# GimpelZhang/GaussianRPG

Measured on AMD Instinct MI355X. Metric: frames/sec @1920x1280, ~2M Gaussians; achieved HBM GB/s vs peak, higher is better.
Workload: dtype f32; 1 GPU; configs[2]: scene-002-like synthetic street scene (seed 2), forward op + clamp + uint8 pack per frame, 200-pose drive, frames sharded round-robin over ranks; P=2000000, width=1920, height=1280, sh_degree=1, M=4, S=0, streams_per_gpu=3, binning_mode=speculative, binning_algorithm=hierarchical, entry_point=GaussianRasterizer.forward, deferred_count=False, frames_rendered_twice=0, parallelism=replicas x1, frame-sharded, final uint8 gather

## Files before the change

### gaussianrpg_amd/csrc/api.hip

```cpp
#include <hip/hip_runtime.h>

#include <atomic>
#include <cmath>
#include <sys/syscall.h>
#include <unistd.h>

#include <cstdio>
#include <cstdlib>
#include <cstring>
#include <mutex>
#include <string>
#include <functional>
#include <vector>

#include "../../include/grpg_rasterizer.h"
#include "abi_util.h"
#include "common.h"

using namespace grpg;

static thread_local std::string g_last_error;

namespace grpg {

// ... 206 lines not shown

int check_async_error(HostWord* hw) {
  if (hw && hw->host_ptr[3] != 0u) {
    hw->host_ptr[3] = 0u;
    return fail(GRPG_ERR_HIP, "render: a producer/consumer hand-over timed out in an earlier frame "
                              "of this thread (image blob header pc_timeout): that frame's image is invalid");
  }
  return GRPG_OK;
}

std::atomic<int> g_binning_alg{[] {
  const char* e = getenv("GRPG_BINNING");
  return (e && strcmp(e, "sort") == 0) ? GRPG_BINNING_ALG_SORT : GRPG_BINNING_ALG_HIER;
}()};
bool binning_is_hier() { return g_binning_alg.load() == GRPG_BINNING_ALG_HIER; }

int bits_for(uint32_t T) {
  int b = 0;
  while ((1ull << b) < (unsigned long long)T) b++;
  return b;
}

struct TimingRecord {
  hipEvent_t ev[GRPG_NUM_STAGES + 1];
  int stage_of[GRPG_NUM_STAGES + 1];
  int n = 0;
};
thread_local std::vector<TimingRecord*> g_pending;
thread_local std::vector<TimingRecord*> g_free;

// ... 413 lines not shown
  uint32_t* const tiles_sorted = (uint32_t*)(geom + GL.tiles_sorted);
  uint32_t* const emit_win = (uint32_t*)(geom + GL.emit_win);
  uint2* const rect_sorted = (uint2*)(geom + GL.rect_sorted);
  uint4* const pre_counts = (uint4*)(geom + GL.pre_counts);
  BlobHeader* const gh = (BlobHeader*)geom;
  uint2* const ranges = (uint2*)(img + IL.ranges);
  uint32_t* const n_contrib = (uint32_t*)(img + IL.n_contrib);
  uint32_t* const work = (uint32_t*)(img + IL.work);

  const bool spec_mode = g_binning_mode.load() == GRPG_BINNING_SPECULATIVE;
  const bool fat_sort = depth_sort_is_fat(GL.nchunks_ds);
  const uint32_t NS = super_tiles(cam.gx, cam.gy);
  const bool hier = fat_sort && binning_is_hier() && NS <= 65536u;
  const bool rect_sorted_by_sort = hier && cam.gx <= 255 && cam.gy <= 255;
  uint2* const rects = hier ? (uint2*)(geom + GL.rects) : nullptr;
  const bool with_ckpt = training && q.S == 0;
  const LayerArgs* const layers = q.layers;
  unsigned char* const tile_obj = layers ? (unsigned char*)(img + IL.ck_count) : nullptr;
  const uint32_t tile_obj_words = layers ? (T + 3u) / 4u : 0u;
  const TileClasses frame_classes = layers ? tile_classes_layers(tile_obj, cam.gx) : tile_classes(q.S);
  const LayerMarks marks = {layers ? layers->layer_class : nullptr, tile_obj, cam.gx};

  const FrameEpilogue* epi = q.epi;
  FrameEpilogue epi_drained;
  uint32_t drain_cnt_words = 0u;
  StageTimer tm{stream, g_timing_enabled};

  HostWord* hw = nullptr;
  uint32_t* pub_ptr = nullptr;
  const uint32_t* pub_host = nullptr;
  hipEvent_t pub_ev = nullptr;
  CapKey ck{-1, 0, 0, 0};
  bool speculative = false;
  bool with_pass3 = true;
  char* bin = nullptr;
// ... 83 lines not shown
    launch_compose_features(stream, q.P, seg_dev, fdev, q.nseg, q.feat_S, q.feat_normals, q.cam_pos,
                            (float*)(q.feat_blob + FL.features));
    return GRPG_OK;
  }

  int enqueue_head() {
    tm.mark(0);
    launch_frame_init(stream, geom, bin, img, (uint32_t)q.P, fat_sort ? 0u : (uint32_t)q.P, Rcap,
                      (uint32_t)q.width, (uint32_t)q.height, (uint32_t)q.S, ranges, T, work,
                      geom + GL.zero_begin, GL.zero_end - GL.zero_begin, training,
                      drain_cnt_words ? (uint32_t*)(img + IL.ck_count) : (uint32_t*)tile_obj,
                      drain_cnt_words ? T + drain_cnt_words : tile_obj_words);
    if (q.segs == nullptr) {
      launch_preprocess(stream, q.P, q.D, q.M, q.means3D, q.scales, q.scale_modifier, q.rotations, q.opacities,
                        q.shs, q.cov3D_precomp, q.colors_precomp, cam, radii_int, rec_w, key_a, tiles, rects,
                        fat_sort ? ds_table : nullptr, pre_counts, marks);
    } else {
      SegmentDev* seg_dev = (SegmentDev*)(geom + GL.seg_table);
      if (int rc = stage_segments(seg_dev)) return rc;
      launch_preprocess_composed(stream, q.P, q.D, q.M, seg_dev, q.nseg, q.scale_modifier, cam, radii_int, rec_w,
                                 key_a, tiles, rects, fat_sort ? ds_table : nullptr, pre_counts, marks);
      if (q.S > 0) {
        if (int rc = stage_features(seg_dev)) return rc;
      }
    }
    const bool fold_publish = fat_sort;
    if (!fold_publish) {
      launch_publish_counts(stream, pre_counts, (uint32_t)((q.P + 255) / 256), pub_ptr, &gh->R_pre);
      HIP_TRY(hipEventRecord(pub_ev, stream));
    }
    STAGE_CHECK("preprocess");
    tm.mark(1);
    if (fat_sort) {
      const uint32_t pnb = (uint32_t)((q.P + 255) / 256);
      uint32_t* key_c = (uint32_t*)(geom + GL.key_c);
      uint32_t* val_c = (uint32_t*)(geom + GL.val_c);
// ... 992 lines not shown
                      const char* binning_buffer, const char* image_buffer, uint64_t* keys_sorted,
                      uint32_t* point_list, uint32_t* ranges, uint32_t* n_contrib, float* means2D,
                      float* depths, float* conic_opacity, float* rgb, uint32_t* tiles_touched,
                      void* hip_stream) {
  if (int rc = begin_call()) return rc;
  if (P < 0 || R < 0 || !geom_buffer || !binning_buffer || !image_buffer)
    return fail(GRPG_ERR_INVALID_ARGUMENT, "bad argument");
  hipStream_t stream = (hipStream_t)hip_stream;
  const int gx = (width + TILE - 1) / TILE, gy = (height + TILE - 1) / TILE;
  const GeomLayout GL = geom_layout((size_t)P);
  BlobHeader bh;
  HIP_TRY(hipMemcpyAsync(&bh, binning_buffer, sizeof(BlobHeader), hipMemcpyDeviceToHost, stream));
  HIP_TRY(hipStreamSynchronize(stream));
  if (bh.magic != BIN_MAGIC || bh.Rcap < (uint32_t)R)
    return fail(GRPG_ERR_BAD_BUFFER, "binning buffer does not match this call");
  const BinLayout BL = bh.hier ? bin_layout((size_t)bh.Rcap, (size_t)gx * gy, super_tiles(gx, gy), (size_t)bh.Rc)
                               : bin_layout((size_t)bh.Rcap);
  const ImgLayout IL = img_layout((size_t)gx * gy, (size_t)width * height);
  launch_debug_export(stream, P, (uint32_t)R, width, height, gx, gy,
                      RecView{(const float4*)(geom_buffer + GL.rec)},
                      (const uint32_t*)(geom_buffer + GL.tiles),
                      (const uint32_t*)(binning_buffer + BL.key_a),
                      bh.hier ? (const uint32_t*)(binning_buffer + BL.tile_start) : nullptr,
                      (const uint32_t*)(binning_buffer + BL.val_a),
                      (const uint2*)(image_buffer + IL.ranges),
                      (const uint32_t*)(image_buffer + IL.n_contrib), keys_sorted, point_list,
                      ranges, n_contrib, means2D, depths, conic_opacity, rgb, tiles_touched);
  HIP_TRY(hipGetLastError());
  return GRPG_OK;
}

}
```

### gaussianrpg_amd/csrc/blend_math.h

```cpp
#pragma once
#include "common.h"

namespace grpg {

typedef float v2f __attribute__((ext_vector_type(2)));

constexpr float LOG2E = 1.4426950408889634f;
constexpr float ALPHA_MIN = 1.0f / 255.0f;
constexpr float ALPHA_MAX = 0.99f;

struct SplatQ {
  float A, B, C;
};

__device__ __forceinline__ SplatQ splat_q(const float cx, const float cy, const float cz) {
  SplatQ q;
  q.A = (-0.5f * LOG2E) * cx;
  q.B = (-LOG2E) * cy;
  q.C = (-0.5f * LOG2E) * cz;
  return q;
}

__device__ __forceinline__ bool splat_power_never_positive(const SplatQ q) {
  const float a = -q.A, c = -q.C;
// ... 55 lines not shown
    const float q2 = c * dyl * dyl + (2.0f * b * dyl + a * dx0) * dx0;
    const float q3 = c * dyh * dyh + (2.0f * b * dyh + a * dx1) * dx1;
    qmin = fminf(fminf(q0, q1), fminf(q2, q3));
  }
  const float thr = 2.0f * __logf(255.0f * opacity);
  const bool far = qmin > thr + 1e-4f * fabsf(thr) + 1e-3f * (1.0f + fabsf(qmin) * 1e-3f);
  const bool transparent = opacity < (1.0f / 255.0f) * 0.999f;
  const bool sane = (a > 0.0f) && (c > 0.0f) && (qmin == qmin) && (opacity == opacity);
  return transparent || (sane && !centre_inside && far);
}

struct QuarterPre {
  float b, ic, det, ct, xtop;
  bool sane, transparent;
};
__device__ __forceinline__ QuarterPre quarter_pre(const float a, const float b, const float c,
                                                  const float opacity) {
  QuarterPre q;
  float t = 2.0f * __logf(255.0f * opacity);
  t = t + 1e-4f * fabsf(t) + 2e-3f;
  const float p = b * b;
  const float det = fmaf(a, c, -p) - fmaf(b, b, -p);
  q.sane = (a > 0.0f) && (c > 0.0f) && (det > 0.0f) && (fabsf(t) < 3e38f) && (fabsf(det) < 3e38f);
  const float ytop = __builtin_amdgcn_sqrtf(fmaxf(t * a * __builtin_amdgcn_rcpf(det), 0.0f));
  q.xtop = -(b * __builtin_amdgcn_rcpf(a)) * ytop;
  q.ct = c * t;
  q.ic = __builtin_amdgcn_rcpf(c);
  q.b = b;
  q.det = det;
  q.transparent = opacity < (1.0f / 255.0f) * 0.999f;
  return q;
}
__device__ __forceinline__ void strip_extent(const QuarterPre& q, const float gx, const float x0,
                                             float& ylo, float& yup, bool& empty) {
  const float xl = x0 - gx, xh = xl + 15.0f;
  const float xet = fminf(fmaxf(q.xtop, xl), xh), xeb = fminf(fmaxf(-q.xtop, xl), xh);
  const float dt = fmaf(-q.det * xet, xet, q.ct), db = fmaf(-q.det * xeb, xeb, q.ct);
  yup = (__builtin_amdgcn_sqrtf(fmaxf(dt, 0.0f)) - q.b * xet) * q.ic;
  ylo = (-__builtin_amdgcn_sqrtf(fmaxf(db, 0.0f)) - q.b * xeb) * q.ic;
  yup += 1e-3f + 1e-5f * fabsf(yup);
  ylo -= 1e-3f + 1e-5f * fabsf(ylo);
  empty = (dt < 0.0f) && (db < 0.0f);
}
__device__ __forceinline__ uint32_t quarter_bits(const bool sane, const bool transparent,
                                                 const float ylo, const float yup, const bool empty,
// ... 34 lines not shown
```

### gaussianrpg_amd/csrc/common.h

```cpp
#pragma once
#include <hip/hip_runtime.h>
#include <stddef.h>
#include <stdint.h>

namespace grpg {

constexpr int TILE = 16;
constexpr int STILE = 8;
constexpr int STILE_TILES = STILE * STILE;
constexpr int WAVE = 64;
constexpr uint32_t CULLED_KEY = 0xFFFFFFFFu;

constexpr uint32_t ID_MASK = 0x0FFFFFFFu;
constexpr int SUBTILE_SHIFT = 28;

constexpr uint32_t REC_CLASS_BIT = 1u << 30;
constexpr uint32_t POINT_CLASS_BIT = 1u << 27;
constexpr int REC_F4 = 3;
constexpr int REC_STRIDE = 4;
struct RecView {
  const float4* rec;
  __device__ __forceinline__ float4 geo0(const size_t id) const { return rec[REC_STRIDE * id]; }
  __device__ __forceinline__ float4 geo1(const size_t id) const { return rec[REC_STRIDE * id + 1]; }
  __device__ __forceinline__ float4 colour(const size_t id) const { return rec[REC_STRIDE * id + 2]; }
// ... 215 lines not shown
}

constexpr uint32_t RENDER_PC_MIN = 8192, RENDER_C1_MIN = 2048, RENDER_HEAVY_MIN = 256;
constexpr int RENDER_NSEM = 16;
static_assert(RENDER_HEAVY_MIN <= CK_LONG_MIN, "lists with blend checkpoints must take the heavy path");
struct TileObjBits {
  const unsigned char* flags;
  int gx;
  __host__ __device__ bool tile(const uint32_t t) const { return flags[t] != 0; }
};
constexpr uint32_t LAYERS_PC_MIN = 4096;
struct TileClasses { uint32_t c0_min, c1_min, heavy_min; TileObjBits obj; uint32_t c0_obj_min; };
inline TileClasses tile_classes(int S) {
  return TileClasses{RENDER_PC_MIN, RENDER_C1_MIN, S > 0 ? 1u : RENDER_HEAVY_MIN, TileObjBits{nullptr, 0}, RENDER_PC_MIN};
}
inline TileClasses tile_classes_layers(const unsigned char* obj_flags, int gx) {
  return TileClasses{RENDER_PC_MIN, RENDER_C1_MIN, RENDER_HEAVY_MIN, TileObjBits{obj_flags, gx}, LAYERS_PC_MIN};
}
__host__ __device__ inline int tile_class(const uint32_t len, const TileClasses tc) {
  return len >= tc.c0_min ? 0 : (len >= tc.c1_min ? 1 : (len >= tc.heavy_min ? 2 : 3));
}
__host__ __device__ inline int tile_class_of(const uint32_t t, const uint32_t len, const TileClasses tc) {
  if (tc.obj.flags == nullptr || len == 0u || !tc.obj.tile(t)) return tile_class(len, tc);
  return len >= tc.c0_obj_min ? 0 : (len >= tc.c1_min ? 1 : 2);
}
struct LayerMarks {
  const unsigned char* layer_class;
  unsigned char* tile_obj;
  int gx;
};
// ... 2 lines not shown
  const float* view;
  const float* proj;
  const float* campos;
  int W, H, gx, gy;
  float tan_fovx, tan_fovy, focal_x, focal_y;
};

void launch_preprocess(hipStream_t s, int P, int D, int M, const float* means3D,
                       const float* scales, float scale_modifier, const float* rotations,
                       const float* opacities, const float* shs, const float* cov3D_precomp,
                       const float* colors_precomp, const CameraArgs& cam, int* radii,
                       float4* rec, uint32_t* depth_key, uint32_t* tiles,
                       uint2* rects ,
                       uint32_t* ds_table0 ,
                       uint4* pre_counts ,
                       LayerMarks lm = LayerMarks{nullptr, nullptr, 0} );
void launch_publish_counts(hipStream_t s, const uint4* pre_counts, uint32_t nblocks,
                           uint32_t* host_word, uint32_t* header_words);
void launch_preprocess_composed(hipStream_t s, int P, int D, int M, const SegmentDev* segs, int nseg,
                                float scale_modifier, const CameraArgs& cam, int* radii, float4* rec,
                                uint32_t* depth_key, uint32_t* tiles, uint2* rects,
                                uint32_t* ds_table0, uint4* pre_counts, LayerMarks lm = LayerMarks{nullptr, nullptr, 0});
void launch_compose(hipStream_t s, int P, int M, const SegmentDev* segs, int nseg, float* means3D,
                    float* scales, float* rotations, float* opacities, float* shs);
void launch_visible_filter(hipStream_t s, int P, const float* means3D, const float* scales,
                           float scale_modifier, const float* rotations,
                           const float* cov3D_precomp, const CameraArgs& cam, int* radii,
                           float* means2D);
void launch_mark_visible(hipStream_t s, int P, const float* means3D, const float* view,
                         unsigned char* present);

bool radix_sort_pairs(hipStream_t s, uint32_t n, const uint32_t* n_dev, uint32_t* key_a,
                      uint32_t* val_a, uint32_t* key_b, uint32_t* val_b, bool vals_iota,
                      int begin_bit, int end_bit, uint32_t* table, uint32_t* totals,
                      uint32_t nchunks, bool have_hist0, const uint32_t* gather_src = nullptr,
                      uint32_t* gather_dst = nullptr);
int radix_sort_num_passes(int begin_bit, int end_bit);
// ... 220 lines not shown
```

### gaussianrpg_amd/csrc/preprocess.hip

```cpp
#include "common.h"

#pragma clang fp contract(off)

#include "gaussian_math.h"
#include "compose_math.h"

namespace grpg {

__device__ __forceinline__ bool project_and_bound(const int idx, const float mx, const float my,
                                                  const float mz, const float s0, const float s1,
                                                  const float s2, const float scale_modifier,
                                                  const float* __restrict__ rotations,
                                                  const float* __restrict__ cov3D_precomp,
                                                  const float* __restrict__ view,
                                                  const float* __restrict__ proj, const int W,
                                                  const int H, const int gx, const int gy,
                                                  const float tan_fovx, const float tan_fovy,
                                                  const float focal_x, const float focal_y,
                                                  Projected& o, const bool q_given = false,
                                                  const float4 q_val = make_float4(1.f, 0.f, 0.f, 0.f)) {
  const float hx = proj[0] * mx + proj[4] * my + proj[8] * mz + proj[12];
  const float hy = proj[1] * mx + proj[5] * my + proj[9] * mz + proj[13];
  const float hw = proj[3] * mx + proj[7] * my + proj[11] * mz + proj[15];
  const float p_w = 1.0f / (hw + 0.0000001f);
// ... 103 lines not shown
    if (w >= 64) {
      for (int ty = 0; ty < h; ty++)
        for (int tx = lane; tx < w; tx += 64) lm.tile_obj[(size_t)(y0 + ty) * lm.gx + x0 + tx] = 1;
    } else {
      const int n = w * h;
      for (int i = lane; i < n; i += 64) {
        int ty = (int)((float)i * __builtin_amdgcn_rcpf((float)w));
        ty -= (ty * w > i) ? 1 : 0;
        ty += ((ty + 1) * w <= i) ? 1 : 0;
        lm.tile_obj[(size_t)(y0 + ty) * lm.gx + x0 + (i - ty * w)] = 1;
      }
    }
  }
}

template <bool HOT>
__global__ void __launch_bounds__(256, HOT ? 8 : 1)
preprocess_kernel(const int P, const int D, const int M, const float* __restrict__ means3D,
                  const float* __restrict__ scales, const float scale_modifier,
                  const float* __restrict__ rotations, const float* __restrict__ opacities,
                  const float* __restrict__ shs, const float* __restrict__ cov3D_precomp,
                  const float* __restrict__ colors_precomp, const float* __restrict__ view,
                  const float* __restrict__ proj, const float* __restrict__ campos, const int W,
                  const int H, const int gx, const int gy, const float tan_fovx,
                  const float tan_fovy, const float focal_x, const float focal_y,
                  int* __restrict__ radii, float4* __restrict__ rec,
                  uint32_t* __restrict__ depth_key, uint32_t* __restrict__ tiles,
                  uint2* __restrict__ rects ,
                  uint32_t* __restrict__ ds_table0 ,
                  uint4* __restrict__ pre_counts ,
                  const int vec_ok_in , const LayerMarks lm) {
  const bool vec_ok = HOT || vec_ok_in != 0;
  const bool has_scales = HOT || scales != nullptr;
  const bool has_cov = !HOT && cov3D_precomp != nullptr;
  const bool has_colors = !HOT && colors_precomp != nullptr;
  const bool layered = !HOT && lm.tile_obj != nullptr;
  __shared__ float4 s_out[256 * REC_STRIDE];
  float* const s_mean = reinterpret_cast<float*>(s_out);
  float* const s_scale = s_mean + 256 * 3;
  const int base = blockIdx.x * 256;
  const int nval = min(256, P - base) * 3;
  {
    const int t4 = threadIdx.x * 4;
    if (vec_ok && t4 + 3 < nval) {
      reinterpret_cast<float4*>(s_mean)[threadIdx.x] =
          reinterpret_cast<const float4*>(means3D + (size_t)base * 3)[threadIdx.x];
// ... 26 lines not shown
  __syncthreads();
  if (idx < P) {
    const bool sh_fast = HOT || (!has_colors && M == 4 && vec_ok);
    float4 q0 = make_float4(0.f, 0.f, 0.f, 0.f), q1 = q0, q2 = q0;
    if (sh_fast) {
      const float4* sp = reinterpret_cast<const float4*>(shs + (size_t)idx * 12);
      q0 = sp[0]; q1 = sp[1]; q2 = sp[2];
    }
    const float opac = opacities[idx];
    const bool q_early = !has_cov;
    const float4 quat = q_early ? load_quat(rotations, idx) : make_float4(1.f, 0.f, 0.f, 0.f);
    Projected o;
    const bool vis = project_and_bound(idx, mx, my, mz, s0, s1, s2, scale_modifier, rotations,
                                       has_cov ? cov3D_precomp : nullptr, view, proj, W, H, gx, gy,
                                       tan_fovx, tan_fovy, focal_x, focal_y, o, q_early, quat);
    if (!vis) {
      radii[idx] = 0;
      tiles[idx] = 0;
      depth_key[idx] = CULLED_KEY;
    } else {
      float rgb[3];
      uint32_t clamped = 0;
      if (!has_colors) {
        const float dx = mx - campos[0];
        const float dy = my - campos[1];
        const float dz = mz - campos[2];
        if (sh_fast) {
          const float sh12[12] = {q0.x, q0.y, q0.z, q0.w, q1.x, q1.y, q1.z, q1.w, q2.x, q2.y, q2.z, q2.w};
          sh_to_rgb(D > 1 ? 1 : D, sh12, dx, dy, dz, rgb, clamped);
        } else {
          sh_to_rgb(D, shs + (size_t)idx * M * 3, dx, dy, dz, rgb, clamped);
        }
      } else {
        rgb[0] = colors_precomp[3 * idx];
        rgb[1] = colors_precomp[3 * idx + 1];
        rgb[2] = colors_precomp[3 * idx + 2];
      }
      radii[idx] = o.radius;
      my_tiles = (uint32_t)(o.maxy - o.miny) * (uint32_t)(o.maxx - o.minx);
      tiles[idx] = my_tiles;
      if (HOT || rects) {
        const uint2 rc = make_uint2((uint32_t)o.minx | ((uint32_t)o.maxx << 16),
                                    (uint32_t)o.miny | ((uint32_t)o.maxy << 16));
        rects[idx] = rc;
        my_st = rect_super_tiles(rc.x, rc.y);
      }
      uint32_t cls_bit = 0u;
      if (layered && lm.layer_class[idx] != 0) {
        if (my_tiles <= (uint32_t)MARK_SMALL) mark_object_tiles(lm, o.minx, o.miny, o.maxx, o.maxy);
        else { mark_big = true; mark_rect = MarkRect{o.minx, o.miny, o.maxx, o.maxy}; }
        cls_bit = REC_CLASS_BIT;
      }
      depth_key[idx] = __float_as_uint(o.depth);
      my_key = __float_as_uint(o.depth);
      r0 = make_float4(o.px, o.py, opac, __uint_as_float((uint32_t)o.radius | cls_bit));
      r1 = make_float4(o.conic[0], o.conic[1], o.conic[2], o.depth);
      r2 = make_float4(rgb[0], rgb[1], rgb[2], __uint_as_float(clamped));
    }
  }
  if (layered) mark_object_tiles_wave(lm, mark_big, mark_rect);
  s_out[REC_STRIDE * threadIdx.x + 0] = r0;
  s_out[REC_STRIDE * threadIdx.x + 1] = r1;
  s_out[REC_STRIDE * threadIdx.x + 2] = r2;
  s_out[REC_STRIDE * threadIdx.x + 3] = make_float4(0.f, 0.f, 0.f, 0.f);
  __syncthreads();
// ... 4 lines not shown
  for (int k = 0; k < REC_STRIDE; k++) {
    const int e = k * 256 + threadIdx.x;
    if (e < nrec4 && __float_as_int(s_out[e & ~(REC_STRIDE - 1)].w) != 0) dst[e] = s_out[e];
  }
  if (HOT || ds_table0 != nullptr) {
    __syncthreads();
#pragma unroll
    for (int k = 0; k < DS_RADIX / 256; k++) {
      const uint32_t cnt = s_dh[k * 256 + threadIdx.x];
      if (cnt != 0u)
        atomicAdd(&ds_table0[(size_t)(blockIdx.x / (DS_CHUNK / 256)) * DS_RADIX + k * 256 + threadIdx.x], cnt);
    }
  }
  if (HOT || pre_counts != nullptr) block_count_sums(my_tiles, my_st, my_key, pre_counts);
}

__global__ void __launch_bounds__(256)
visible_filter_kernel(const int P, const float* __restrict__ means3D,
                      const float* __restrict__ scales, const float scale_modifier,
                      const float* __restrict__ rotations,
                      const float* __restrict__ cov3D_precomp, const float* __restrict__ view,
                      const float* __restrict__ proj, const int W, const int H, const int gx,
                      const int gy, const float tan_fovx, const float tan_fovy,
                      const float focal_x, const float focal_y, int* __restrict__ radii,
                      float* __restrict__ means2D) {
  const int idx = blockIdx.x * 256 + threadIdx.x;
  if (idx >= P) return;
  Projected o;
  const bool has_s = scales != nullptr;
  const bool vis = project_and_bound(idx, means3D[3 * idx], means3D[3 * idx + 1],
// ... 30 lines not shown
  const uint32_t j = (uint32_t)idx - sg.start;
  const Activated a = compose_one(sg, j);
  means3D[3 * idx] = a.mx; means3D[3 * idx + 1] = a.my; means3D[3 * idx + 2] = a.mz;
  scales[3 * idx] = a.s0; scales[3 * idx + 1] = a.s1; scales[3 * idx + 2] = a.s2;
  rotations[4 * idx] = a.q.x; rotations[4 * idx + 1] = a.q.y; rotations[4 * idx + 2] = a.q.z;
  rotations[4 * idx + 3] = a.q.w;
  opacities[idx] = a.opacity;
  float* o = shs + (size_t)idx * M * 3;
  o[0] = a.dc[0]; o[1] = a.dc[1]; o[2] = a.dc[2];
  if (M > 1) {
    const float* fr = sg.frest + (size_t)j * (M - 1) * 3;
    for (int k = 0; k < (M - 1) * 3; k++) o[3 + k] = fr[k];
  }
}

template <bool M4, bool HOT>
__global__ void __launch_bounds__(256, HOT ? 8 : 1)
preprocess_composed_kernel(const int P, const int D, const int M,
                           const SegmentDev* __restrict__ segs, const int nseg,
                           const float scale_modifier, const float* __restrict__ view,
                           const float* __restrict__ proj, const float* __restrict__ campos,
                           const int W, const int H, const int gx, const int gy,
                           const float tan_fovx, const float tan_fovy, const float focal_x,
                           const float focal_y, int* __restrict__ radii, float4* __restrict__ rec,
                           uint32_t* __restrict__ depth_key, uint32_t* __restrict__ tiles,
                           uint2* __restrict__ rects, uint32_t* __restrict__ ds_table0,
                           uint4* __restrict__ pre_counts, const LayerMarks lm) {
  static_assert(M4 || !HOT, "the specialised instantiation keeps its four SH coefficients in registers");
  const bool layered = !HOT && lm.tile_obj != nullptr;
  __shared__ float4 s_out[256 * REC_STRIDE];
  __shared__ uint32_t s_dh[DS_RADIX];
#pragma unroll
  for (int k = 0; k < DS_RADIX / 256; k++) s_dh[k * 256 + threadIdx.x] = 0u;
  const int base = blockIdx.x * 256;
  const int idx = base + threadIdx.x;
  float4 r0 = make_float4(0.f, 0.f, 0.f, 0.f), r1 = r0, r2 = r0;
  uint32_t my_key = CULLED_KEY, my_tiles = 0u, my_st = 0u;
  bool mark_big = false;
  MarkRect mark_rect = {0, 0, 0, 0};
  if (idx < P) {
    const SegmentDev& sg = *find_segment(segs, nseg, (uint32_t)idx);
    const uint32_t j = (uint32_t)idx - sg.start;
    const Activated a = compose_one(sg, j);
    Projected o;
    const bool vis = project_and_bound(idx, a.mx, a.my, a.mz, a.s0, a.s1, a.s2, scale_modifier,
                                       nullptr, nullptr, view, proj, W, H, gx, gy, tan_fovx, tan_fovy,
                                       focal_x, focal_y, o, true, a.q);
    if (!vis) {
      radii[idx] = 0;
      tiles[idx] = 0;
      depth_key[idx] = CULLED_KEY;
    } else {
      float rgb[3];
      uint32_t clamped = 0;
      const float dx = a.mx - campos[0];
      const float dy = a.my - campos[1];
      const float dz = a.mz - campos[2];
      if (M4) {
        const float* fr = sg.frest + (size_t)j * 9;
        const float sh12[12] = {a.dc[0], a.dc[1], a.dc[2], fr[0], fr[1], fr[2], fr[3], fr[4], fr[5],
                                fr[6], fr[7], fr[8]};
        sh_to_rgb(D > 1 ? 1 : D, sh12, dx, dy, dz, rgb, clamped);
      } else {
        float sh[48];
        compose_features(sg, j, a, M, sh);
        sh_to_rgb(D, sh, dx, dy, dz, rgb, clamped);
      }
      radii[idx] = o.radius;
      my_tiles = (uint32_t)(o.maxy - o.miny) * (uint32_t)(o.maxx - o.minx);
      tiles[idx] = my_tiles;
      if (HOT || rects) {
        const uint2 rc = make_uint2((uint32_t)o.minx | ((uint32_t)o.maxx << 16),
                                    (uint32_t)o.miny | ((uint32_t)o.maxy << 16));
        rects[idx] = rc;
        my_st = rect_super_tiles(rc.x, rc.y);
      }
      uint32_t cls_bit = 0u;
      if (layered && ((uint32_t)(uintptr_t)sg.pad1 & 1u)) {
        if (my_tiles <= (uint32_t)MARK_SMALL) mark_object_tiles(lm, o.minx, o.miny, o.maxx, o.maxy);
        else { mark_big = true; mark_rect = MarkRect{o.minx, o.miny, o.maxx, o.maxy}; }
        cls_bit = REC_CLASS_BIT;
      }
      depth_key[idx] = __float_as_uint(o.depth);
      my_key = __float_as_uint(o.depth);
      r0 = make_float4(o.px, o.py, a.opacity, __uint_as_float((uint32_t)o.radius | cls_bit));
      r1 = make_float4(o.conic[0], o.conic[1], o.conic[2], o.depth);
      r2 = make_float4(rgb[0], rgb[1], rgb[2], __uint_as_float(clamped));
    }
  }
  if (layered) mark_object_tiles_wave(lm, mark_big, mark_rect);
  s_out[REC_STRIDE * threadIdx.x + 0] = r0;
  s_out[REC_STRIDE * threadIdx.x + 1] = r1;
  s_out[REC_STRIDE * threadIdx.x + 2] = r2;
  s_out[REC_STRIDE * threadIdx.x + 3] = make_float4(0.f, 0.f, 0.f, 0.f);
  __syncthreads();
// ... 4 lines not shown
  for (int k = 0; k < REC_STRIDE; k++) {
    const int e = k * 256 + threadIdx.x;
    if (e < nrec4 && __float_as_int(s_out[e & ~(REC_STRIDE - 1)].w) != 0) dst[e] = s_out[e];
  }
  if (HOT || ds_table0 != nullptr) {
    __syncthreads();
#pragma unroll
    for (int k = 0; k < DS_RADIX / 256; k++) {
      const uint32_t cnt = s_dh[k * 256 + threadIdx.x];
      if (cnt != 0u)
        atomicAdd(&ds_table0[(size_t)(blockIdx.x / (DS_CHUNK / 256)) * DS_RADIX + k * 256 + threadIdx.x], cnt);
    }
  }
  if (HOT || pre_counts != nullptr) block_count_sums(my_tiles, my_st, my_key, pre_counts);
}

void launch_preprocess_composed(hipStream_t s, int P, int D, int M, const SegmentDev* segs, int nseg,
                                float scale_modifier, const CameraArgs& cam, int* radii, float4* rec,
                                uint32_t* depth_key, uint32_t* tiles, uint2* rects,
                                uint32_t* ds_table0, uint4* pre_counts, LayerMarks lm) {
  if (P <= 0) return;
#define PC_LAUNCH(M4, HOT)                                                                      \
  preprocess_composed_kernel<M4, HOT><<<(P + 255) / 256, 256, 0, s>>>(                           \
      P, D, M, segs, nseg, scale_modifier, cam.view, cam.proj, cam.campos, cam.W, cam.H, cam.gx,  \
      cam.gy, cam.tan_fovx, cam.tan_fovy, cam.focal_x, cam.focal_y, radii, rec, depth_key, tiles, \
      rects, ds_table0, pre_counts, lm)
  const bool hot = M == 4 && lm.tile_obj == nullptr && rects != nullptr && ds_table0 != nullptr &&
                   pre_counts != nullptr;
  if (hot) PC_LAUNCH(true, true); else if (M == 4) PC_LAUNCH(true, false); else PC_LAUNCH(false, false);
#undef PC_LAUNCH
}

void launch_compose(hipStream_t s, int P, int M, const SegmentDev* segs, int nseg, float* means3D,
                    float* scales, float* rotations, float* opacities, float* shs) {
  if (P <= 0) return;
  compose_kernel<<<(P + 255) / 256, 256, 0, s>>>(P, M, segs, nseg, means3D, scales, rotations,
                                                  opacities, shs);
}

void launch_preprocess(hipStream_t s, int P, int D, int M, const float* means3D,
                       const float* scales, float scale_modifier, const float* rotations,
                       const float* opacities, const float* shs, const float* cov3D_precomp,
                       const float* colors_precomp, const CameraArgs& cam, int* radii,
                       float4* rec, uint32_t* depth_key, uint32_t* tiles, uint2* rects,
                       uint32_t* ds_table0, uint4* pre_counts, LayerMarks lm) {
  if (P <= 0) return;
  const int vec_ok = ((((uintptr_t)means3D | (uintptr_t)scales | (uintptr_t)shs) & 15) == 0) ? 1 : 0;
  const bool hot = cov3D_precomp == nullptr && colors_precomp == nullptr && scales != nullptr && M == 4 && vec_ok &&
                   lm.tile_obj == nullptr && rects != nullptr && ds_table0 != nullptr && pre_counts != nullptr;
#define PP_LAUNCH(HOT)                                                                              \
  preprocess_kernel<HOT><<<(P + 255) / 256, 256, 0, s>>>(                                            \
      P, D, M, means3D, scales, scale_modifier, rotations, opacities, shs, cov3D_precomp,            \
      colors_precomp, cam.view, cam.proj, cam.campos, cam.W, cam.H, cam.gx, cam.gy, cam.tan_fovx,    \
      cam.tan_fovy, cam.focal_x, cam.focal_y, radii, rec, depth_key, tiles, rects, ds_table0,        \
      pre_counts, vec_ok, lm)
  if (hot) PP_LAUNCH(true); else PP_LAUNCH(false);
#undef PP_LAUNCH
}

void launch_visible_filter(hipStream_t s, int P, const float* means3D, const float* scales,
                           float scale_modifier, const float* rotations,
                           const float* cov3D_precomp, const CameraArgs& cam, int* radii,
                           float* means2D) {
  if (P <= 0) return;
  visible_filter_kernel<<<(P + 255) / 256, 256, 0, s>>>(
      P, means3D, scales, scale_modifier, rotations, cov3D_precomp, cam.view, cam.proj, cam.W,
      cam.H, cam.gx, cam.gy, cam.tan_fovx, cam.tan_fovy, cam.focal_x, cam.focal_y, radii, means2D);
}

void launch_mark_visible(hipStream_t s, int P, const float* means3D, const float* view,
                         unsigned char* present) {
// ... 6 lines not shown
```

### gaussianrpg_amd/csrc/render_fwd.hip

```cpp
#include "blend_math.h"
#include "common.h"
#include "sky_math.h"

namespace grpg {

constexpr int RW_WAVES = 4;

constexpr int NUM_CLASSES = 4;

__global__ void __launch_bounds__(256)
classify_tiles_kernel(const uint32_t T, const uint2* __restrict__ ranges, const TileClasses tc,
                      uint32_t* __restrict__ work) {
  const uint32_t t = blockIdx.x * 256 + threadIdx.x;
  const uint32_t lane = threadIdx.x & 63;
  int cls = -1;
  if (t < T) {
    const uint2 r = ranges[t];
    const uint32_t len = r.y - r.x;
    cls = tile_class_of(t, len, tc);
  }
#pragma unroll
  for (int c = 0; c < NUM_CLASSES; c++) {
    const uint64_t m = __ballot(cls == c);
    if (m == 0ull) continue;
// ... 1616 lines not shown
  }
}

uint32_t render_pc_slots(uint32_t R) { return 2u * (uint32_t)((size_t)R / RENDER_PC_MIN + 1); }

void launch_render_forward(hipStream_t s, const uint2* ranges, const uint32_t* point_list,
                           const RecView rec, int W, int H, int gx, int gy, const float* bg,
                           float* out_color, float* out_depth, float* out_alpha,
                           uint32_t* n_contrib, uint32_t* work ,
                           const TileClasses cls, uint32_t R, bool aux, bool classified,
                           const CkptArgs* ckp, const PCErr pc_err, const float* semantics, int S,
                           float* out_semantic, const FrameEpilogue* epi) {
  const int ntiles = gx * gy;
  if (ntiles <= 0) return;
  const CkptArgs ck = (aux && ckp) ? *ckp : CkptArgs{nullptr, nullptr, nullptr, nullptr, 0u, 0u};
  const uint32_t pc_slots = render_pc_slots(R);
  if (!classified)
    classify_tiles_kernel<<<(ntiles + 255) / 256, 256, 0, s>>>((uint32_t)ntiles, ranges, cls, work);
  const SemSrc sem = {semantics, S, nullptr};
#define RF_ARGS ranges, point_list, rec, W, H, gx, (uint32_t)ntiles, work, bg, out_color, out_depth, \
                out_alpha, n_contrib, pc_slots, ck, pc_err, sem, out_semantic
  if (epi != nullptr && !aux && S == 0) {
    const FrameEpi fe = make_frame_epi(epi, W, true);
    render_forward_kernel<false, 2, 0, false, true><<<ntiles + pc_slots + fe.drain_wgs, 256, 0, s>>>(
        RF_ARGS, LayerOut{nullptr, nullptr, nullptr, nullptr, nullptr}, TileObjBits{nullptr, 0}, fe);
  } else if (S > 0) {
    if (aux) render_forward_kernel<true, 2, RENDER_NSEM><<<ntiles + pc_slots, 256, 0, s>>>(RF_ARGS);
    else render_forward_kernel<false, 2, RENDER_NSEM><<<ntiles + pc_slots, 256, 0, s>>>(RF_ARGS);
  } else {
    if (aux) render_forward_kernel<true, 2><<<ntiles + pc_slots, 256, 0, s>>>(RF_ARGS);
    else render_forward_kernel<false, 1><<<ntiles + pc_slots, 256, 0, s>>>(RF_ARGS);
// ... 30 lines not shown
```

Baseline: 2726 frames/s.

## Bin Gaussians by tight alpha-threshold ellipse box instead of radius rect

In inference with hierarchical binning, preprocess computes a tile box from the conic and opacity where alpha reaches 1/255, and intersects it with the radius-based rect before writing rects. Fully transparent or empty-box Gaussians get a culled depth key, so they never enter the sort or the tile lists. This cuts tile/Gaussian pairs and blending work. Because binned tiles now carry fewer entries, the tile-class thresholds are scaled down by 11/16 and pc_slots is derived from the class threshold. The risks are extra per-Gaussian math in preprocess and subtle differences at ellipse edges.

```diff
diff --git a/gaussianrpg_amd/csrc/api.hip b/gaussianrpg_amd/csrc/api.hip
--- a/gaussianrpg_amd/csrc/api.hip
+++ b/gaussianrpg_amd/csrc/api.hip
@@ -244,6 +244,10 @@
   return (e && strcmp(e, "sort") == 0) ? GRPG_BINNING_ALG_SORT : GRPG_BINNING_ALG_HIER;
 }()};
 bool binning_is_hier() { return g_binning_alg.load() == GRPG_BINNING_ALG_HIER; }
+bool alpha_rect_enabled() {
+  static const bool on = [] { const char* v = getenv("GRPG_ALPHA_RECT"); return !(v && atoi(v) == 0); }();
+  return on;
+}
 
 int bits_for(uint32_t T) {
   int b = 0;
@@ -687,11 +691,13 @@
   const bool hier = fat_sort && binning_is_hier() && NS <= 65536u;
   const bool rect_sorted_by_sort = hier && cam.gx <= 255 && cam.gy <= 255;
   uint2* const rects = hier ? (uint2*)(geom + GL.rects) : nullptr;
+  const bool binned_rects = hier && !training && alpha_rect_enabled();
   const bool with_ckpt = training && q.S == 0;
   const LayerArgs* const layers = q.layers;
   unsigned char* const tile_obj = layers ? (unsigned char*)(img + IL.ck_count) : nullptr;
   const uint32_t tile_obj_words = layers ? (T + 3u) / 4u : 0u;
-  const TileClasses frame_classes = layers ? tile_classes_layers(tile_obj, cam.gx) : tile_classes(q.S);
+  const TileClasses frame_classes = layers ? tile_classes_layers(tile_obj, cam.gx)
+                                           : (binned_rects ? tile_classes_binned(q.S) : tile_classes(q.S));
   const LayerMarks marks = {layers ? layers->layer_class : nullptr, tile_obj, cam.gx};
 
   const FrameEpilogue* epi = q.epi;
@@ -805,12 +811,12 @@
     if (q.segs == nullptr) {
       launch_preprocess(stream, q.P, q.D, q.M, q.means3D, q.scales, q.scale_modifier, q.rotations, q.opacities,
                         q.shs, q.cov3D_precomp, q.colors_precomp, cam, radii_int, rec_w, key_a, tiles, rects,
-                        fat_sort ? ds_table : nullptr, pre_counts, marks);
+                        fat_sort ? ds_table : nullptr, pre_counts, marks, binned_rects);
     } else {
       SegmentDev* seg_dev = (SegmentDev*)(geom + GL.seg_table);
       if (int rc = stage_segments(seg_dev)) return rc;
       launch_preprocess_composed(stream, q.P, q.D, q.M, seg_dev, q.nseg, q.scale_modifier, cam, radii_int, rec_w,
-                                 key_a, tiles, rects, fat_sort ? ds_table : nullptr, pre_counts, marks);
+                                 key_a, tiles, rects, fat_sort ? ds_table : nullptr, pre_counts, marks, binned_rects);
       if (q.S > 0) {
         if (int rc = stage_features(seg_dev)) return rc;
       }
@@ -1833,10 +1839,15 @@
   HIP_TRY(hipStreamSynchronize(stream));
   if (bh.magic != BIN_MAGIC || bh.Rcap < (uint32_t)R)
     return fail(GRPG_ERR_BAD_BUFFER, "binning buffer does not match this call");
+  BlobHeader gh;
+  HIP_TRY(hipMemcpyAsync(&gh, geom_buffer, sizeof(BlobHeader), hipMemcpyDeviceToHost, stream));
+  HIP_TRY(hipStreamSynchronize(stream));
+  if (gh.magic != GEOM_MAGIC) return fail(GRPG_ERR_BAD_BUFFER, "geometry buffer does not match this call");
+  const uint32_t R_listed = bh.hier && gh.R < (uint32_t)R ? gh.R : (uint32_t)R;
   const BinLayout BL = bh.hier ? bin_layout((size_t)bh.Rcap, (size_t)gx * gy, super_tiles(gx, gy), (size_t)bh.Rc)
                                : bin_layout((size_t)bh.Rcap);
   const ImgLayout IL = img_layout((size_t)gx * gy, (size_t)width * height);
-  launch_debug_export(stream, P, (uint32_t)R, width, height, gx, gy,
+  launch_debug_export(stream, P, R_listed, width, height, gx, gy,
                       RecView{(const float4*)(geom_buffer + GL.rec)},
                       (const uint32_t*)(geom_buffer + GL.tiles),
                       (const uint32_t*)(binning_buffer + BL.key_a),
diff --git a/gaussianrpg_amd/csrc/blend_math.h b/gaussianrpg_amd/csrc/blend_math.h
--- a/gaussianrpg_amd/csrc/blend_math.h
+++ b/gaussianrpg_amd/csrc/blend_math.h
@@ -93,21 +93,57 @@
   float b, ic, det, ct, xtop;
   bool sane, transparent;
 };
+struct AlphaEllipse {
+  float t, det;
+  bool sane, transparent;
+};
+__device__ __forceinline__ AlphaEllipse alpha_ellipse(const float a, const float b, const float c,
+                                                      const float opacity) {
+  AlphaEllipse e;
+  float t = 2.0f * __logf(255.0f * opacity);
+  t = t + 1e-4f * fabsf(t) + 2e-3f;
+  const float p = b * b;
+  e.det = fmaf(a, c, -p) - fmaf(b, b, -p);
+  e.t = t;
+  e.sane = (a > 0.0f) && (c > 0.0f) && (e.det > 0.0f) && (fabsf(t) < 3e38f) && (fabsf(e.det) < 3e38f);
+  e.transparent = opacity < (1.0f / 255.0f) * 0.999f;
+  return e;
+}
+struct AlphaBox {
+  int x0, x1, y0, y1;
+  bool keep_all, transparent;
+};
+__device__ __forceinline__ AlphaBox alpha_box(const float px, const float py, const float a, const float b,
+                                              const float c, const float opacity) {
+  const AlphaEllipse e = alpha_ellipse(a, b, c, opacity);
+  const float s = e.t * __builtin_amdgcn_rcpf(e.det);
+  float hx = __builtin_amdgcn_sqrtf(fmaxf(s * c, 0.0f)), hy = __builtin_amdgcn_sqrtf(fmaxf(s * a, 0.0f));
+  hx += 1e-3f + 1e-5f * fabsf(hx);
+  hy += 1e-3f + 1e-5f * fabsf(hy);
+  const float fx0 = ceilf((px - hx - 15.0f) * 0.0625f), fx1 = floorf((px + hx) * 0.0625f);
+  const float fy0 = ceilf((py - hy - 15.0f) * 0.0625f), fy1 = floorf((py + hy) * 0.0625f);
+  AlphaBox o;
+  const bool finite = fabsf(fx0) < 1048576.0f && fabsf(fx1) < 1048576.0f && fabsf(fy0) < 1048576.0f &&
+                      fabsf(fy1) < 1048576.0f;
+  o.keep_all = !e.sane || !finite;
+  o.transparent = e.transparent;
+  o.x0 = (int)fx0; o.x1 = (int)fx1 + 1;
+  o.y0 = (int)fy0; o.y1 = (int)fy1 + 1;
+  return o;
+}
 __device__ __forceinline__ QuarterPre quarter_pre(const float a, const float b, const float c,
                                                   const float opacity) {
   QuarterPre q;
-  float t = 2.0f * __logf(255.0f * opacity);
-  t = t + 1e-4f * fabsf(t) + 2e-3f;
-  const float p = b * b;
-  const float det = fmaf(a, c, -p) - fmaf(b, b, -p);
-  q.sane = (a > 0.0f) && (c > 0.0f) && (det > 0.0f) && (fabsf(t) < 3e38f) && (fabsf(det) < 3e38f);
+  const AlphaEllipse e = alpha_ellipse(a, b, c, opacity);
+  const float t = e.t, det = e.det;
+  q.sane = e.sane;
   const float ytop = __builtin_amdgcn_sqrtf(fmaxf(t * a * __builtin_amdgcn_rcpf(det), 0.0f));
   q.xtop = -(b * __builtin_amdgcn_rcpf(a)) * ytop;
   q.ct = c * t;
   q.ic = __builtin_amdgcn_rcpf(c);
   q.b = b;
   q.det = det;
-  q.transparent = opacity < (1.0f / 255.0f) * 0.999f;
+  q.transparent = e.transparent;
   return q;
 }
 __device__ __forceinline__ void strip_extent(const QuarterPre& q, const float gx, const float x0,
diff --git a/gaussianrpg_amd/csrc/common.h b/gaussianrpg_amd/csrc/common.h
--- a/gaussianrpg_amd/csrc/common.h
+++ b/gaussianrpg_amd/csrc/common.h
@@ -253,6 +253,14 @@
 inline TileClasses tile_classes(int S) {
   return TileClasses{RENDER_PC_MIN, RENDER_C1_MIN, S > 0 ? 1u : RENDER_HEAVY_MIN, TileObjBits{nullptr, 0}, RENDER_PC_MIN};
 }
+constexpr uint32_t BINNED_CLASS_NUM = 11, BINNED_CLASS_DEN = 16;
+inline TileClasses tile_classes_binned(int S) {
+  TileClasses c = tile_classes(S);
+  c.c0_min = c.c0_obj_min = RENDER_PC_MIN * BINNED_CLASS_NUM / BINNED_CLASS_DEN;
+  c.c1_min = RENDER_C1_MIN * BINNED_CLASS_NUM / BINNED_CLASS_DEN;
+  if (S == 0) c.heavy_min = RENDER_HEAVY_MIN * BINNED_CLASS_NUM / BINNED_CLASS_DEN;
+  return c;
+}
 inline TileClasses tile_classes_layers(const unsigned char* obj_flags, int gx) {
   return TileClasses{RENDER_PC_MIN, RENDER_C1_MIN, RENDER_HEAVY_MIN, TileObjBits{obj_flags, gx}, LAYERS_PC_MIN};
 }
@@ -285,13 +293,15 @@
                        uint2* rects ,
                        uint32_t* ds_table0 ,
                        uint4* pre_counts ,
-                       LayerMarks lm = LayerMarks{nullptr, nullptr, 0} );
+                       LayerMarks lm = LayerMarks{nullptr, nullptr, 0} ,
+                       bool binned = false );
 void launch_publish_counts(hipStream_t s, const uint4* pre_counts, uint32_t nblocks,
                            uint32_t* host_word, uint32_t* header_words);
 void launch_preprocess_composed(hipStream_t s, int P, int D, int M, const SegmentDev* segs, int nseg,
                                 float scale_modifier, const CameraArgs& cam, int* radii, float4* rec,
                                 uint32_t* depth_key, uint32_t* tiles, uint2* rects,
-                                uint32_t* ds_table0, uint4* pre_counts, LayerMarks lm = LayerMarks{nullptr, nullptr, 0});
+                                uint32_t* ds_table0, uint4* pre_counts, LayerMarks lm = LayerMarks{nullptr, nullptr, 0},
+                                bool binned = false );
 void launch_compose(hipStream_t s, int P, int M, const SegmentDev* segs, int nseg, float* means3D,
                     float* scales, float* rotations, float* opacities, float* shs);
 void launch_visible_filter(hipStream_t s, int P, const float* means3D, const float* scales,
diff --git a/gaussianrpg_amd/csrc/preprocess.hip b/gaussianrpg_amd/csrc/preprocess.hip
--- a/gaussianrpg_amd/csrc/preprocess.hip
+++ b/gaussianrpg_amd/csrc/preprocess.hip
@@ -4,6 +4,7 @@
 
 #include "gaussian_math.h"
 #include "compose_math.h"
+#include "blend_math.h"
 
 namespace grpg {
 
@@ -141,22 +142,34 @@
   }
 }
 
-template <bool HOT>
-__global__ void __launch_bounds__(256, HOT ? 8 : 1)
-preprocess_kernel(const int P, const int D, const int M, const float* __restrict__ means3D,
-                  const float* __restrict__ scales, const float scale_modifier,
-                  const float* __restrict__ rotations, const float* __restrict__ opacities,
-                  const float* __restrict__ shs, const float* __restrict__ cov3D_precomp,
-                  const float* __restrict__ colors_precomp, const float* __restrict__ view,
-                  const float* __restrict__ proj, const float* __restrict__ campos, const int W,
-                  const int H, const int gx, const int gy, const float tan_fovx,
-                  const float tan_fovy, const float focal_x, const float focal_y,
-                  int* __restrict__ radii, float4* __restrict__ rec,
-                  uint32_t* __restrict__ depth_key, uint32_t* __restrict__ tiles,
-                  uint2* __restrict__ rects ,
-                  uint32_t* __restrict__ ds_table0 ,
-                  uint4* __restrict__ pre_counts ,
-                  const int vec_ok_in , const LayerMarks lm) {
+#define PP_PARAMS                                                                                                  \
+  const int P, const int D, const int M, const float* __restrict__ means3D, const float* __restrict__ scales,      \
+      const float scale_modifier, const float* __restrict__ rotations, const float* __restrict__ opacities,        \
+      const float* __restrict__ shs, const float* __restrict__ cov3D_precomp,                                      \
+      const float* __restrict__ colors_precomp, const float* __restrict__ view, const float* __restrict__ proj,    \
+      const float* __restrict__ campos, const int W, const int H, const int gx, const int gy,                      \
+      const float tan_fovx, const float tan_fovy, const float focal_x, const float focal_y,                        \
+      int* __restrict__ radii, float4* __restrict__ rec, uint32_t* __restrict__ depth_key,                         \
+      uint32_t* __restrict__ tiles, uint2* __restrict__ rects, uint32_t* __restrict__ ds_table0,                   \
+      uint4* __restrict__ pre_counts, const int vec_ok_in, const LayerMarks lm
+#define PP_ARGS                                                                                                    \
+  P, D, M, means3D, scales, scale_modifier, rotations, opacities, shs, cov3D_precomp, colors_precomp, view, proj,  \
+      campos, W, H, gx, gy, tan_fovx, tan_fovy, focal_x, focal_y, radii, rec, depth_key, tiles, rects, ds_table0,  \
+      pre_counts, vec_ok_in, lm
+
+struct TileRect { int minx, miny, maxx, maxy; };
+__device__ __forceinline__ bool binned_rect(const Projected& o, const float opacity, TileRect& r) {
+  r = TileRect{o.minx, o.miny, o.maxx, o.maxy};
+  const AlphaBox ab = alpha_box(o.px, o.py, o.conic[0], o.conic[1], o.conic[2], opacity);
+  if (!ab.keep_all) {
+    r.minx = max(r.minx, ab.x0); r.maxx = min(r.maxx, ab.x1);
+    r.miny = max(r.miny, ab.y0); r.maxy = min(r.maxy, ab.y1);
+  }
+  return !ab.transparent && r.maxx > r.minx && r.maxy > r.miny;
+}
+
+template <bool HOT, bool BINNED>
+__device__ __forceinline__ void preprocess_body(PP_PARAMS) {
   const bool vec_ok = HOT || vec_ok_in != 0;
   const bool has_scales = HOT || scales != nullptr;
   const bool has_cov = !HOT && cov3D_precomp != nullptr;
@@ -213,11 +226,19 @@
     const bool vis = project_and_bound(idx, mx, my, mz, s0, s1, s2, scale_modifier, rotations,
                                        has_cov ? cov3D_precomp : nullptr, view, proj, W, H, gx, gy,
                                        tan_fovx, tan_fovy, focal_x, focal_y, o, q_early, quat);
+    TileRect br = {0, 0, 0, 0};
+    const bool binned = vis && (BINNED ? binned_rect(o, opac, br) : true);
     if (!vis) {
       radii[idx] = 0;
       tiles[idx] = 0;
       depth_key[idx] = CULLED_KEY;
+    } else if (BINNED && !binned) {
+      radii[idx] = o.radius;
+      my_tiles = (uint32_t)(o.maxy - o.miny) * (uint32_t)(o.maxx - o.minx);
+      tiles[idx] = my_tiles;
+      depth_key[idx] = CULLED_KEY;
     } else {
+      if (!BINNED) br = TileRect{o.minx, o.miny, o.maxx, o.maxy};
       float rgb[3];
       uint32_t clamped = 0;
       if (!has_colors) {
@@ -239,15 +260,16 @@
       my_tiles = (uint32_t)(o.maxy - o.miny) * (uint32_t)(o.maxx - o.minx);
       tiles[idx] = my_tiles;
       if (HOT || rects) {
-        const uint2 rc = make_uint2((uint32_t)o.minx | ((uint32_t)o.maxx << 16),
-                                    (uint32_t)o.miny | ((uint32_t)o.maxy << 16));
+        const uint2 rc = make_uint2((uint32_t)br.minx | ((uint32_t)br.maxx << 16),
+                                    (uint32_t)br.miny | ((uint32_t)br.maxy << 16));
         rects[idx] = rc;
         my_st = rect_super_tiles(rc.x, rc.y);
       }
       uint32_t cls_bit = 0u;
       if (layered && lm.layer_class[idx] != 0) {
-        if (my_tiles <= (uint32_t)MARK_SMALL) mark_object_tiles(lm, o.minx, o.miny, o.maxx, o.maxy);
-        else { mark_big = true; mark_rect = MarkRect{o.minx, o.miny, o.maxx, o.maxy}; }
+        if ((uint32_t)(br.maxy - br.miny) * (uint32_t)(br.maxx - br.minx) <= (uint32_t)MARK_SMALL)
+          mark_object_tiles(lm, br.minx, br.miny, br.maxx, br.maxy);
+        else { mark_big = true; mark_rect = MarkRect{br.minx, br.miny, br.maxx, br.maxy}; }
         cls_bit = REC_CLASS_BIT;
       }
       depth_key[idx] = __float_as_uint(o.depth);
@@ -282,6 +304,16 @@
   }
   if (HOT || pre_counts != nullptr) block_count_sums(my_tiles, my_st, my_key, pre_counts);
 }
+template <bool HOT>
+__global__ void __launch_bounds__(256, HOT ? 8 : 1) preprocess_kernel(PP_PARAMS) {
+  preprocess_body<HOT, false>(PP_ARGS);
+}
+template <bool HOT>
+__global__ void __launch_bounds__(256, HOT ? 8 : 1) preprocess_binned_kernel(PP_PARAMS) {
+  preprocess_body<HOT, true>(PP_ARGS);
+}
+#undef PP_PARAMS
+#undef PP_ARGS
 
 __global__ void __launch_bounds__(256)
 visible_filter_kernel(const int P, const float* __restrict__ means3D,
@@ -342,18 +374,19 @@
   }
 }
 
-template <bool M4, bool HOT>
-__global__ void __launch_bounds__(256, HOT ? 8 : 1)
-preprocess_composed_kernel(const int P, const int D, const int M,
-                           const SegmentDev* __restrict__ segs, const int nseg,
-                           const float scale_modifier, const float* __restrict__ view,
-                           const float* __restrict__ proj, const float* __restrict__ campos,
-                           const int W, const int H, const int gx, const int gy,
-                           const float tan_fovx, const float tan_fovy, const float focal_x,
-                           const float focal_y, int* __restrict__ radii, float4* __restrict__ rec,
-                           uint32_t* __restrict__ depth_key, uint32_t* __restrict__ tiles,
-                           uint2* __restrict__ rects, uint32_t* __restrict__ ds_table0,
-                           uint4* __restrict__ pre_counts, const LayerMarks lm) {
+#define PC_PARAMS                                                                                                 \
+  const int P, const int D, const int M, const SegmentDev* __restrict__ segs, const int nseg,                     \
+      const float scale_modifier, const float* __restrict__ view, const float* __restrict__ proj,                 \
+      const float* __restrict__ campos, const int W, const int H, const int gx, const int gy,                     \
+      const float tan_fovx, const float tan_fovy, const float focal_x, const float focal_y,                       \
+      int* __restrict__ radii, float4* __restrict__ rec, uint32_t* __restrict__ depth_key,                        \
+      uint32_t* __restrict__ tiles, uint2* __restrict__ rects, uint32_t* __restrict__ ds_table0,                  \
+      uint4* __restrict__ pre_counts, const LayerMarks lm
+#define PC_ARGS                                                                                                   \
+  P, D, M, segs, nseg, scale_modifier, view, proj, campos, W, H, gx, gy, tan_fovx, tan_fovy, focal_x, focal_y,    \
+      radii, rec, depth_key, tiles, rects, ds_table0, pre_counts, lm
+template <bool M4, bool HOT, bool BINNED>
+__device__ __forceinline__ void preprocess_composed_body(PC_PARAMS) {
   static_assert(M4 || !HOT, "the specialised instantiation keeps its four SH coefficients in registers");
   const bool layered = !HOT && lm.tile_obj != nullptr;
   __shared__ float4 s_out[256 * REC_STRIDE];
@@ -374,11 +407,19 @@
     const bool vis = project_and_bound(idx, a.mx, a.my, a.mz, a.s0, a.s1, a.s2, scale_modifier,
                                        nullptr, nullptr, view, proj, W, H, gx, gy, tan_fovx, tan_fovy,
                                        focal_x, focal_y, o, true, a.q);
+    TileRect br = {0, 0, 0, 0};
+    const bool binned = vis && (BINNED ? binned_rect(o, a.opacity, br) : true);
     if (!vis) {
       radii[idx] = 0;
       tiles[idx] = 0;
       depth_key[idx] = CULLED_KEY;
+    } else if (BINNED && !binned) {
+      radii[idx] = o.radius;
+      my_tiles = (uint32_t)(o.maxy - o.miny) * (uint32_t)(o.maxx - o.minx);
+      tiles[idx] = my_tiles;
+      depth_key[idx] = CULLED_KEY;
     } else {
+      if (!BINNED) br = TileRect{o.minx, o.miny, o.maxx, o.maxy};
       float rgb[3];
       uint32_t clamped = 0;
       const float dx = a.mx - campos[0];
@@ -398,15 +439,16 @@
       my_tiles = (uint32_t)(o.maxy - o.miny) * (uint32_t)(o.maxx - o.minx);
       tiles[idx] = my_tiles;
       if (HOT || rects) {
-        const uint2 rc = make_uint2((uint32_t)o.minx | ((uint32_t)o.maxx << 16),
-                                    (uint32_t)o.miny | ((uint32_t)o.maxy << 16));
+        const uint2 rc = make_uint2((uint32_t)br.minx | ((uint32_t)br.maxx << 16),
+                                    (uint32_t)br.miny | ((uint32_t)br.maxy << 16));
         rects[idx] = rc;
         my_st = rect_super_tiles(rc.x, rc.y);
       }
       uint32_t cls_bit = 0u;
       if (layered && ((uint32_t)(uintptr_t)sg.pad1 & 1u)) {
-        if (my_tiles <= (uint32_t)MARK_SMALL) mark_object_tiles(lm, o.minx, o.miny, o.maxx, o.maxy);
-        else { mark_big = true; mark_rect = MarkRect{o.minx, o.miny, o.maxx, o.maxy}; }
+        if ((uint32_t)(br.maxy - br.miny) * (uint32_t)(br.maxx - br.minx) <= (uint32_t)MARK_SMALL)
+          mark_object_tiles(lm, br.minx, br.miny, br.maxx, br.maxy);
+        else { mark_big = true; mark_rect = MarkRect{br.minx, br.miny, br.maxx, br.maxy}; }
         cls_bit = REC_CLASS_BIT;
       }
       depth_key[idx] = __float_as_uint(o.depth);
@@ -441,20 +483,38 @@
   }
   if (HOT || pre_counts != nullptr) block_count_sums(my_tiles, my_st, my_key, pre_counts);
 }
+template <bool M4, bool HOT>
+__global__ void __launch_bounds__(256, HOT ? 8 : 1) preprocess_composed_kernel(PC_PARAMS) {
+  preprocess_composed_body<M4, HOT, false>(PC_ARGS);
+}
+template <bool M4, bool HOT>
+__global__ void __launch_bounds__(256, HOT ? 8 : 1) preprocess_composed_binned_kernel(PC_PARAMS) {
+  preprocess_composed_body<M4, HOT, true>(PC_ARGS);
+}
+#undef PC_PARAMS
+#undef PC_ARGS
 
 void launch_preprocess_composed(hipStream_t s, int P, int D, int M, const SegmentDev* segs, int nseg,
                                 float scale_modifier, const CameraArgs& cam, int* radii, float4* rec,
                                 uint32_t* depth_key, uint32_t* tiles, uint2* rects,
-                                uint32_t* ds_table0, uint4* pre_counts, LayerMarks lm) {
+                                uint32_t* ds_table0, uint4* pre_counts, LayerMarks lm, bool binned) {
   if (P <= 0) return;
-#define PC_LAUNCH(M4, HOT)                                                                      \
-  preprocess_composed_kernel<M4, HOT><<<(P + 255) / 256, 256, 0, s>>>(                           \
+#define PC_LAUNCH(KERNEL, M4, HOT)                                                              \
+  KERNEL<M4, HOT><<<(P + 255) / 256, 256, 0, s>>>(                                                \
       P, D, M, segs, nseg, scale_modifier, cam.view, cam.proj, cam.campos, cam.W, cam.H, cam.gx,  \
       cam.gy, cam.tan_fovx, cam.tan_fovy, cam.focal_x, cam.focal_y, radii, rec, depth_key, tiles, \
       rects, ds_table0, pre_counts, lm)
   const bool hot = M == 4 && lm.tile_obj == nullptr && rects != nullptr && ds_table0 != nullptr &&
                    pre_counts != nullptr;
-  if (hot) PC_LAUNCH(true, true); else if (M == 4) PC_LAUNCH(true, false); else PC_LAUNCH(false, false);
+  if (binned && rects != nullptr) {
+    if (hot) PC_LAUNCH(preprocess_composed_binned_kernel, true, true);
+    else if (M == 4) PC_LAUNCH(preprocess_composed_binned_kernel, true, false);
+    else PC_LAUNCH(preprocess_composed_binned_kernel, false, false);
+  } else {
+    if (hot) PC_LAUNCH(preprocess_composed_kernel, true, true);
+    else if (M == 4) PC_LAUNCH(preprocess_composed_kernel, true, false);
+    else PC_LAUNCH(preprocess_composed_kernel, false, false);
+  }
 #undef PC_LAUNCH
 }
 
@@ -470,18 +530,22 @@
                        const float* opacities, const float* shs, const float* cov3D_precomp,
                        const float* colors_precomp, const CameraArgs& cam, int* radii,
                        float4* rec, uint32_t* depth_key, uint32_t* tiles, uint2* rects,
-                       uint32_t* ds_table0, uint4* pre_counts, LayerMarks lm) {
+                       uint32_t* ds_table0, uint4* pre_counts, LayerMarks lm, bool binned) {
   if (P <= 0) return;
-  const int vec_ok = ((((uintptr_t)means3D | (uintptr_t)scales | (uintptr_t)shs) & 15) == 0) ? 1 : 0;
+  const int vec_ok =((((uintptr_t)means3D | (uintptr_t)scales | (uintptr_t)shs) & 15) == 0) ? 1 : 0;
   const bool hot = cov3D_precomp == nullptr && colors_precomp == nullptr && scales != nullptr && M == 4 && vec_ok &&
                    lm.tile_obj == nullptr && rects != nullptr && ds_table0 != nullptr && pre_counts != nullptr;
-#define PP_LAUNCH(HOT)                                                                              \
-  preprocess_kernel<HOT><<<(P + 255) / 256, 256, 0, s>>>(                                            \
+#define PP_LAUNCH(KERNEL, HOT)                                                                      \
+  KERNEL<HOT><<<(P + 255) / 256, 256, 0, s>>>(                                                       \
       P, D, M, means3D, scales, scale_modifier, rotations, opacities, shs, cov3D_precomp,            \
       colors_precomp, cam.view, cam.proj, cam.campos, cam.W, cam.H, cam.gx, cam.gy, cam.tan_fovx,    \
       cam.tan_fovy, cam.focal_x, cam.focal_y, radii, rec, depth_key, tiles, rects, ds_table0,        \
       pre_counts, vec_ok, lm)
-  if (hot) PP_LAUNCH(true); else PP_LAUNCH(false);
+  if (binned && rects != nullptr) {
+    if (hot) PP_LAUNCH(preprocess_binned_kernel, true); else PP_LAUNCH(preprocess_binned_kernel, false);
+  } else {
+    if (hot) PP_LAUNCH(preprocess_kernel, true); else PP_LAUNCH(preprocess_kernel, false);
+  }
 #undef PP_LAUNCH
 }
 
diff --git a/gaussianrpg_amd/csrc/render_fwd.hip b/gaussianrpg_amd/csrc/render_fwd.hip
--- a/gaussianrpg_amd/csrc/render_fwd.hip
+++ b/gaussianrpg_amd/csrc/render_fwd.hip
@@ -1654,7 +1654,7 @@
   const int ntiles = gx * gy;
   if (ntiles <= 0) return;
   const CkptArgs ck = (aux && ckp) ? *ckp : CkptArgs{nullptr, nullptr, nullptr, nullptr, 0u, 0u};
-  const uint32_t pc_slots = render_pc_slots(R);
+  const uint32_t pc_slots = 2u * (uint32_t)((size_t)R / cls.c0_min + 1);
   if (!classified)
     classify_tiles_kernel<<<(ntiles + 255) / 256, 256, 0, s>>>((uint32_t)ntiles, ranges, cls, work);
   const SemSrc sem = {semantics, S, nullptr};
```

Result: faster. 2787 frames/s (median of 6 runs) (+2.2%).
